# RoadlyInc/DSOPP

Hardware: AMD Instinct MI355X
Metric: Gauss-Newton iters/sec (7-KF window, 2k active pts) (higher is better)
Workload: dtype f64; 1 GPU; C1: 7-KF window, 2000 active points per GPU (2000 total, 2000 on rank 0), 640x480, full clique, production LM settings; frames=7, points_per_gpu=2000, total_points=2000, parallelism=single GPU, exchange=none, ranks=1

## Files before the change

### dsopp_amd/csrc/pba.hip

```cpp
#include <algorithm>
#include <chrono>
#include <cstdlib>
#include <map>
#include <memory>
#include <mutex>

#include "host_linalg.hpp"
#include "pba_solve_kernels.hpp"
#include "pba_solve_combined.hpp"
#include "pba_schur_two_stage.hpp"
#include "depth_map_kernels.hpp"
#include "point_status_kernels.hpp"
#include "depth_maps.hpp"
#include "activation_kernels.hpp"
#include "immature_set.hpp"
#include "semantic_observation_kernels.hpp"

namespace dsopp_hip {
namespace {

struct ResidualTable {
  DeviceBuffer<uint8_t> status, cand, fej_valid, snap_status;
  DeviceBuffer<double> energy;
  int n = 0, snap_n = 0;
// ... 924 lines not shown
  a.st = w.d_state.ptr;
  const bool combined = fused && fused->combined;
  const size_t reduce_count = combined ? w.combCount() : w.reduceCount();
  a.comb = combined ? w.d_reduce.ptr : nullptr;
  a.comb_lambda = fused ? fused->comb_lambda : 0.0;
  if (combined && mode == ReduceMode::kAccumulateOnly && w.comb_copies_active > 1) {
    a.comb_copies = w.comb_copies_active;
    a.comb_copy_first = static_cast<int>(w.combCopyFirst());
    a.comb_copy_stride = static_cast<int>(w.combCopyStride());
  }
  a.scalars = mode == ReduceMode::kDecideOnly ? w.d_reduce.ptr + reduce_count : w.d_scalars.ptr;
  a.n_sweep_blocks = w.n_sweep_blocks;
  a.total_blocks = a.n_schur_blocks + F * F;
  a.scalars_out = mode == ReduceMode::kAccumulateOnly ? w.d_reduce.ptr + reduce_count : nullptr;
  const bool grouped_tail = mode == ReduceMode::kAccumulateOnly && w.allreduce != nullptr;
  a.scalars_out_groups = grouped_tail ? kScalarGroups : 0;
  static_assert(4 * kScalarGroups <= kSchurThreads, "one workgroup writes the grouped tail");
  if (fused) a.prm = fused->prm;
  if (fused && fused->scalars) a.scalars = fused->scalars;
  a.ctrl_host = fused ? fused->ctrl_host : nullptr;
  a.dbg = w.dbg_stamps ? w.dbg_stamps.get() + 24 : nullptr;
  return a;
}

void launchReduceSchur(W &w, bool for_marg, const LmControl *ctrl, const FusedReduce *fused = nullptr, ReduceMode mode = ReduceMode::kFused) {
  const int K = w.K(), F = w.F();
  hipStream_t st = w.sr.stream;
  if (!fused && !for_marg && !ctrl && w.deterministic) {
    launchTwoStage(w, nullptr, 0, 0.0, true, nullptr);
    allreduceIfNeeded(w, w.d_reduce.ptr, w.reduceCount());
    return;
  }
  ensureDynamicLds(reinterpret_cast<const void *>(reduceSchurKernel), w.sr.device, 96 * 1024);
  const ReduceSchurArgs a = makeReduceSchurArgs(w, for_marg, ctrl, fused, mode);
  const size_t reduce_count = (fused && fused->combined) ? w.combCount() : w.reduceCount();
  const bool grouped_tail = mode == ReduceMode::kAccumulateOnly && w.allreduce != nullptr;
  const size_t decide_smem = kDecideSmemBytes;
  if (mode == ReduceMode::kDecideOnly) {
    timedLaunch(w, DSOPP_HIP_KERNEL_ACCEPT,
                [&] { decideApplyKernel<<<std::max(1, a.n_schur_blocks), kSchurThreads, decide_smem, st>>>(a); });
    HIP_CHECK(hipGetLastError());
    return;
  }
  timedLaunch(w, DSOPP_HIP_KERNEL_SCHUR, [&] {
    reduceSchurKernel<<<a.n_schur_blocks + F * F + (a.scalars_out ? 1 : 0), kSchurThreads, std::max(schurSmemBytes(K), decide_smem), st>>>(
        a.ctrl, a.schur_table, a.pc, a.partials, a.pair_first_block, a.pair_num_blocks, a.n_schur_blocks, a.F, a);
  });
  HIP_CHECK(hipGetLastError());
  allreduceIfNeeded(w, w.d_reduce.ptr, reduce_count + (mode == ReduceMode::kAccumulateOnly ? (grouped_tail ? 4 * kScalarGroups : 4) : 0));
  (void)K;
}

SolveArgs makeSolveArgs(W &w) {
  SolveArgs a;
  a.frames = w.d_frames.ptr;
  a.st = w.d_state.ptr;
  a.pc = w.d_pc.ptr;
  a.Hpp_raw = w.dHppRaw();
  a.bpp_raw = w.dbppRaw();
  a.Hpp_out = w.d_Hpp.ptr;
  a.Hsc_copy = w.d_Hpp.ptr + static_cast<size_t>(w.K()) * w.K();
  a.bpp_out = w.d_bpp.ptr;
  a.Hsc = w.dHsc();
  a.bsc = w.dbsc();
  a.use_marginal = w.marg_nonzero ? 1 : 0;
  a.Hm = w.d_Hm.ptr;
  a.bm = w.d_bm.ptr;
  a.step = w.d_step.ptr;
  a.lambda = 0;
  a.affine_reg[0] = w.opt.affine_brightness_regularizer[0];
  a.affine_reg[1] = w.opt.affine_brightness_regularizer[1];
  a.fixed_reg = w.opt.fixed_state_regularizer;
  a.energy_marginalized = w.energy_marginalized;
  a.F = w.F();
  a.fej = w.fej() ? 1 : 0;
  a.do_solve = 1;
  a.store_system = 0;
  a.add_priors = 1;
  return a;
}

size_t solveSmemBytes(int K) {
  const size_t N = static_cast<size_t>(K) + 1;
  return (N * (N + 1) + 4 * static_cast<size_t>(K) + 32 + 38 * static_cast<size_t>(kMaxFrames)) * sizeof(double);
}

void launchAssemble(W &w, double lambda, bool do_solve, bool add_priors, bool store_system) {
  ensureDynamicLds(reinterpret_cast<const void *>(assembleSolveKernel), w.sr.device, 150 * 1024);
  SolveArgs a = makeSolveArgs(w);
  a.lambda = lambda;
  a.do_solve = do_solve ? 1 : 0;
  a.add_priors = add_priors ? 1 : 0;
  a.store_system = store_system ? 1 : 0;
  timedLaunch(w, do_solve ? DSOPP_HIP_KERNEL_ASSEMBLE_SOLVE : DSOPP_HIP_KERNEL_ASSEMBLE,
              [&] { assembleSolveKernel<<<1, kSolveThreads, solveSmemBytes(w.K()), w.sr.stream>>>(a); });
  if (do_solve && !w.fej()) {
    pairSetupKernel<<<1, kMaxFrames * kMaxFrames, 0, w.sr.stream>>>(w.d_frames.ptr, w.d_state.ptr, w.d_pc.ptr, w.F(), 0, nullptr);
  }
  HIP_CHECK(hipGetLastError());
}

void launchTwoStage(W &w, const LmControl *ctrl, int ublk_parity, double lambda, bool dense = false, double *group_sums = nullptr) {
  const int F = w.F();
  hipStream_t st = w.sr.stream;
  using TwoStageKernel = void (*)(TwoStageArgs);
  static const TwoStageKernel kernels[6] = {nullptr, schurTwoStageKernel<2>, schurTwoStageKernel<2>, schurTwoStageKernel<3>, schurTwoStageKernel<4>,
                                            schurTwoStageKernel<5>};
  const int tpw = twoStageTilesPerWave(F);
  if (tpw < 1 || tpw > kMaxTilesPerWave) fail(DSOPP_HIP_ERR_CAPACITY, "window of %d frames exceeds the Schur kernel's tile budget", F);
  const TwoStageKernel two_stage_kernel = kernels[tpw];
  ensureDynamicLds(reinterpret_cast<const void *>(two_stage_kernel), w.sr.device, 96 * 1024);
  const int n_chunks = w.opt.optimize_idepths ? w.n_schur_blocks : 0;
  const int n_wgs = std::max(1, std::min(512, n_chunks));
  w.d_schur_partials.reserve(std::max<size_t>(1, static_cast<size_t>(n_wgs)) * static_cast<size_t>(twoStagePartialCount(F)), 0, st);
  w.d_pair_out.reserve(static_cast<size_t>(kMaxFrames) * kMaxFrames * kPairOut, 0, st);
  TwoStageArgs a;
  a.frames = w.d_frames.ptr;
  a.pc = w.d_pc.ptr;
  a.schur_table = w.d_schur_table.ptr;
  a.partials = w.d_partials.ptr;
  a.dbg = w.dbg_stamps ? w.dbg_stamps.get() + 32 : nullptr;
  a.pair_first_block = w.d_pair_first.ptr;
  a.pair_num_blocks = w.d_pair_count.ptr;
  a.ctrl = ctrl;
  a.schur_partials = w.d_schur_partials.ptr;
  a.pair_out = w.d_pair_out.ptr;
  a.F = F;
  a.n_chunks = n_chunks;
  a.n_schur_wgs = n_wgs;
  a.ublk_parity = ublk_parity;
  a.group_sums = group_sums;
  a.n_sweep_blocks = w.n_sweep_blocks;
  CombineArgs c;
  c.pc = w.d_pc.ptr;
  c.schur_partials = w.d_schur_partials.ptr;
  c.pair_out = w.d_pair_out.ptr;
  c.ctrl = ctrl;
  c.lambda = lambda;
  c.comb = w.d_reduce.ptr;
  c.dense = dense ? w.d_reduce.ptr : nullptr;
  c.F = F;
  c.n_schur_wgs = n_wgs;
  const size_t pair_smem = (48 + 64 + kPairBlk + 8 * 48) * sizeof(double);
  timedLaunch(w, DSOPP_HIP_KERNEL_SCHUR, [&] {
    two_stage_kernel<<<n_wgs + F * F + (group_sums ? kScalarGroups : 0), kSchurThreads, std::max(twoStageSmemBytes(F), pair_smem), st>>>(a);
    combineSystemKernel<<<static_cast<unsigned>((twoStagePartialCount(F) + kCombineEntries - 1) / kCombineEntries), kCombineEntries * kCombineSlices, 0, st>>>(c);
  });
  HIP_CHECK(hipGetLastError());
}

int solveResidentWorkgroups(W &w, bool wide) {
  static std::map<std::pair<int, size_t>, int> cache;
  static std::mutex mu;
  const size_t smem = solveSmemBytes(w.K());
  std::lock_guard<std::mutex> lock(mu);
  const auto key = std::make_pair(w.sr.device * 2 + (wide ? 1 : 0), smem);
  auto it = cache.find(key);
  if (it != cache.end()) return it->second;
  int per_cu = 0, cus = 0;
  if (wide)
    HIP_CHECK(hipOccupancyMaxActiveBlocksPerMultiprocessor(&per_cu, solveCombinedKernel<512>, 512, smem));
  else
    HIP_CHECK(hipOccupancyMaxActiveBlocksPerMultiprocessor(&per_cu, solveCombinedKernel<256>, 256, smem));
  HIP_CHECK(hipDeviceGetAttribute(&cus, hipDeviceAttributeMultiprocessorCount, w.sr.device));
  const int n = std::max(2, per_cu * cus);
  cache[key] = n;
  return n;
// ... 2688 lines not shown
```

### dsopp_amd/csrc/pba_solve_combined.hpp

```cpp
#pragma once
#include "pba_solve_kernels.hpp"

namespace dsopp_hip {

struct SolveCombArgs {
  const FrameDev *frames;
  WindowState *st;
  PairConst *pc;
  const double *comb;
  int comb_copies = 1;
  int comb_copy_first = 0, comb_copy_stride = 0;
  const double *Hm, *bm;
  const double *HmPacked = nullptr;
  double *step;
  LmControl *ctrl;
  double lambda;
  double affine_reg[2];
  double fixed_reg;
  double energy_marginalized;
  int F;
  int fej;
  int use_marginal;
  long long *dbg_stamps;
  const LmControl *dec_in = nullptr;
  const double *dec_scalars = nullptr;
  const SchurBlock *dec_table = nullptr;
  int dec_blocks = 0;
  int dec_groups = 0;
  LmParams dec_prm;
  unsigned *bs_ticket = nullptr;
  double *bs_hand = nullptr;
  double *bs_hand_next = nullptr;
  int bs_parity = 0;
  int dec_chunks = 0;
  unsigned bs_ticket_base = 0;
  int *bs_fault = nullptr;
  const unsigned *arrive = nullptr;
  unsigned arrive_target = 0;
  int fused_first = 0;
};
__device__ __forceinline__ bool waitForReducers(const unsigned *arrive, unsigned target, bool patient, int *fault) {
  const long long t0 = wall_clock64();
  for (;;) {
    const unsigned v = __hip_atomic_load(glb(arrive), __ATOMIC_RELAXED, __HIP_MEMORY_SCOPE_AGENT);
    if (static_cast<int>(v - target) >= 0) return true;
    if (patient)
      __builtin_amdgcn_s_sleep(24);
    else
      __builtin_amdgcn_s_sleep(1);
    if (wall_clock64() - t0 > 200000000ll) {
      if (fault) __hip_atomic_store(fault, 1, __ATOMIC_RELAXED, __HIP_MEMORY_SCOPE_SYSTEM);
      return false;
    }
  }
}
__host__ __device__ inline double kHandOverSentinel() {
  union {
    unsigned long long u;
    double d;
  } c;
  c.u = 0x7FF8D50FF00DBEEFull;
  return c.d;
}
constexpr int kMaxCombCopies = 4;
#define SC_STAMP(i) do { if (kStamps && a.dbg_stamps && tid == 0) a.dbg_stamps[i] = wall_clock64(); } while (0)

__device__ __forceinline__ void combBlockDecode(int b, int &bi, int &bj) {
  int r = static_cast<int>((__fsqrt_rn(8.0f * static_cast<float>(b) + 1.0f) - 1.0f) * 0.5f);
  if ((r + 1) * (r + 2) / 2 <= b) ++r;
  if (r * (r + 1) / 2 > b) --r;
  bi = r;
  bj = b - r * (r + 1) / 2;
}

template <int THREADS, int COPIES, bool FUSED>
__device__ __forceinline__ void solveCombinedBody(char *smem_raw, unsigned *bs_ticket_p, double *bs_hand_next_p, const LmControl *dec_in_p,
                                                  const double *dec_scalars_p, const double *comb_p, const FrameDev *frames_p, WindowState *st_p,
                                                  int F_p, const SolveCombArgs &a, const double *t_fused) {
  const int F = F_p, K = kBlk * F;
  const int N = K + 1;
  const int ld = N + 1;
  double *A = reinterpret_cast<double *>(smem_raw);
  double *pv = A + N * ld;
  double *xs = pv + K;
  double *Linv = xs + K + 16;
  double *epsl = Linv + 36 * kMaxFrames;
  double *stpl = epsl + K;
  double *ab0l = stpl + K;
  const int tid = threadIdx.x;
  const int wave = tid >> 6, lane = tid & 63;
  const long long sc_t_entry = (kStamps && a.dbg_stamps) ? wall_clock64() : 0;

  int c_active = 1, c_relin = 0;
  double lam = a.lambda;
  const bool decides = dec_in_p != nullptr;
  double dec_eps = 0, dec_step = 0;
  int dec_accept = 0;
  const bool ticketed = FUSED || bs_ticket_p != nullptr;
  const unsigned vblock_f = FUSED ? blockIdx.x - static_cast<unsigned>(a.fused_first) : 0u;
  unsigned ticket_raw = 0;
  if (!FUSED && ticketed && tid == 0) {
    auto tp = glb(bs_ticket_p);
    asm volatile("" : "+v"(tp));
    ticket_raw = __hip_atomic_fetch_add(tp, 1u, __ATOMIC_RELAXED, __HIP_MEMORY_SCOPE_AGENT);
  }
  if (ticketed && tid < kBlk * kMaxFrames) bs_hand_next_p[tid] = kHandOverSentinel();
  const void DSOPP_CONSTANT *any_words = (const void DSOPP_CONSTANT *)__builtin_amdgcn_kernarg_segment_ptr();
  const LmControl DSOPP_CONSTANT *cin_src = dec_in_p ? (const LmControl DSOPP_CONSTANT *)dec_in_p : (const LmControl DSOPP_CONSTANT *)any_words;
  static_assert(sizeof(SolveCombArgs) >= sizeof(LmControl) && sizeof(SolveCombArgs) >= 4 * sizeof(double), "the argument block stands in for an absent control block / scalar block");
  static_assert(sizeof(LmControl) == 6 * sizeof(double) + 8 * sizeof(int), "LmControl changed: extend the scalar copy below");
  LmControl cin;
  cin.lambda = cin_src->lambda;
  cin.energy = cin_src->energy;
  cin.cand_prior = cin_src->cand_prior;
  cin.idepth_sq = cin_src->idepth_sq;
  cin.frame_state_sq = cin_src->frame_state_sq;
  cin.frame_step_sq = cin_src->frame_step_sq;
  cin.n_valid = cin_src->n_valid;
  cin.converged = cin_src->converged;
  cin.active = cin_src->active;
  cin.linear_system_valid = cin_src->linear_system_valid;
  cin.iteration = cin_src->iteration;
  cin.need_final_setup = cin_src->need_final_setup;
  cin.pending = cin_src->pending;
  cin.relin = cin_src->relin;
  const double DSOPP_CONSTANT *t_src =
      (!FUSED && dec_scalars_p) ? (const double DSOPP_CONSTANT *)dec_scalars_p : (const double DSOPP_CONSTANT *)any_words;
  double t_early[4] = {t_src[0], t_src[1], t_src[2], t_src[3]};
  asm volatile("" : "+s"(cin.lambda), "+s"(cin.energy), "+s"(cin.cand_prior), "+s"(cin.idepth_sq), "+s"(cin.frame_state_sq), "+s"(cin.frame_step_sq),
               "+s"(cin.n_valid), "+s"(cin.converged), "+s"(cin.active), "+s"(cin.linear_system_valid), "+s"(cin.iteration),
               "+s"(cin.need_final_setup), "+s"(cin.pending), "+s"(cin.relin), "+s"(t_early[0]), "+s"(t_early[1]), "+s"(t_early[2]), "+s"(t_early[3])
               : "s"(a.pc), "s"(a.Hm), "s"(a.bm), "s"(a.HmPacked), "s"(a.step), "s"(a.ctrl), "s"(a.fej), "s"(a.use_marginal), "s"(a.dec_table),
               "s"(a.dec_blocks), "s"(a.dec_groups), "s"(a.bs_hand), "s"(a.bs_parity), "s"(a.dec_chunks), "s"(a.bs_ticket_base), "s"(a.comb_copies),
               "s"(a.comb_copy_first), "s"(a.comb_copy_stride), "s"(a.lambda), "s"(a.affine_reg[0]), "s"(a.affine_reg[1]), "s"(a.fixed_reg),
               "s"(a.energy_marginalized));
  __shared__ unsigned s_vblock;
  bool main_wg = FUSED ? vblock_f == 0 : (ticketed || blockIdx.x == 0);
  const bool reducers_build = FUSED && cin.active && !cin.linear_system_valid;
  struct {
    int valid;
    Rigid T0;
    double fxr, fyr, cxr, cyr, fxt, fyt, cxt, cyt, exposure_r, exposure_t;
  } pp;
  pp.valid = 0;
  const bool fast_refresh = a.fej != 0;
  auto requestPairInputs = [&] {
    if (fast_refresh && tid < F * F) {
      const int r = tid / F, t = tid - F * (tid / F);
      const PairConst &P = a.pc[r * kMaxFrames + t];
      pp.valid = P.valid;
#pragma unroll
      for (int i = 0; i < 3; ++i) {
#pragma unroll
        for (int j = 0; j < 3; ++j) pp.T0.R[3 * i + j] = P.T0rel[4 * i + j];
        pp.T0.t[i] = P.T0rel[4 * i + 3];
      }
      const FrameDev &fr = frames_p[r];
      const FrameDev &ft = frames_p[t];
      pp.fxr = fr.fx;
      pp.fyr = fr.fy;
      pp.cxr = fr.cx;
      pp.cyr = fr.cy;
      pp.fxt = ft.fx;
      pp.fyt = ft.fy;
      pp.cxt = ft.cx;
      pp.cyt = ft.cy;
      pp.exposure_r = fr.exposure;
      pp.exposure_t = ft.exposure;
    }
  };
  double eps_c = 0, ab0_c = 0, rhs_c = 0, bm_c = 0;
  int fixed_c = 0, tomarg_c = 0;
// ... 227 lines not shown
              break;
            }
          }
        }
        stp[tid] = v;
      }
      __syncthreads();
      if (s_timed_out) return;
      const double damp = 1.0 / (1.0 + s_dec_out.lambda);
      auto finish = [&](const double (&rw)[NS][kBlk], double bd, double ih, hbm_f64 *dst) {
        double d = 0;
    #pragma unroll
        for (int q = 0; q < NS; ++q) {
          const double *sq = stp + kBlk * (sub + 4 * q);
    #pragma unroll
          for (int c = 0; c < kBlk; ++c) d += rw[q][c] * sq[c];
        }
        d += dppMove<0xB1>(d);
        d += dppMove<0x4E>(d);
        if (sub == 0 && dst) *dst = -((bd - d) * damp * ih);
      };
    #pragma unroll
      for (int u = 0; u < kPre; ++u) finish(rows[u], bdv[u], ihv[u], dstp[u]);
      for (int p = static_cast<int>(vblock) - 1 + kPre * W; p < n_pass; p += W) {
        double rw[NS][kBlk], bd = 0, ih = 0;
        hbm_f64 *dst = nullptr;
    #pragma unroll
        for (int q = 0; q < NS; ++q)
    #pragma unroll
          for (int c = 0; c < kBlk; ++c) rw[q][c] = 0;
        fetch(p, rw, bd, ih, dst);
        finish(rw, bd, ih, dst);
      }
      };
      if (THREADS < 512)
        backSubstitute(std::integral_constant<int, 2>{});
      else if (F <= 12)
        backSubstitute(std::integral_constant<int, 3>{});
      else
        backSubstitute(std::integral_constant<int, 4>{});
      return;
    }
    if (cin.pending && tid < K) {
      if (dec_accept) {
        dec_eps += dec_step;
        st_p->eps[tid >> 3][tid & 7] = dec_eps;
      }
      st_p->step[tid >> 3][tid & 7] = 0;
    }
    if (tid == 64) *a.ctrl = s_dec_out;
    if (!s_dec_proceed) return;
    c_active = 1;
    c_relin = s_dec_out.relin;
    lam = s_dec_out.lambda;
  } else if (a.ctrl) {
    c_active = a.ctrl->active;
    c_relin = a.ctrl->relin;
    lam = a.ctrl->lambda;
  }
  if (decides) eps_c = dec_eps;
  SC_STAMP(0);
  if (kStamps && a.dbg_stamps && tid == 0) a.dbg_stamps[7] = sc_t_entry;
  asm volatile("" : "+v"(fixed_c), "+v"(tomarg_c), "+v"(c_active), "+v"(c_relin));
  int prior_kind = 0;
  double pd_c = 0;
  if (tid < K) {
    if (!tomarg_c) prior_kind = fixed_c ? 1 : ((tid & 7) >= 6 ? 2 : 0);
    pd_c = prior_kind == 1 ? a.fixed_reg : (prior_kind == 2 ? ((tid & 7) == 6 ? a.affine_reg[0] : a.affine_reg[1]) : 0.0);
    xs[tid] = eps_c;
    epsl[tid] = eps_c;
    Linv[tid] = pd_c;
    if ((tid & 7) >= 6) ab0l[2 * (tid >> 3) + (tid & 7) - 6] = ab0_c;
  }
  ldsBarrier();
  SC_STAMP(10);
  if (!c_active || c_relin) return;
  if (FUSED) {
    __shared__ int s_system_there;
    if (tid == 0) s_system_there = (!reducers_build || waitForReducers(a.arrive, a.arrive_target, false, a.bs_fault)) ? 1 : 0;
    ldsBarrier();
    if (!s_system_there) return;
    SC_STAMP(16);
    if (tid < K) rhs_c = __hip_atomic_load(glb(comb_p) + combBlockCount(F) * 64 + tid, __ATOMIC_RELAXED, __HIP_MEMORY_SCOPE_AGENT);
    loadBatch(0);
  }
  const double *prior_diag = Linv;
  const int in_row = (tid >> 3) & 7, in_col = tid & 7;
  double *const A_thr = A + in_row * ld + in_col;
  auto storeBatch = [&](int base) {
    int blk = __builtin_amdgcn_readfirstlane((base + tid) >> 6);
    int bi, bj;
    combBlockDecode(blk, bi, bj);
    bi = __builtin_amdgcn_readfirstlane(bi);
    bj = __builtin_amdgcn_readfirstlane(bj);
    const int n_blocks = n_entries >> 6;
#pragma unroll
    for (int u = 0; u < kBatch; ++u) {
      if (blk < n_blocks) {
        const int blk_off = __builtin_amdgcn_readfirstlane(8 * bi * ld + 8 * bj);
        const double v = hv[u] + hm[u];
        if (bi != bj) {
          A_thr[blk_off] = v;
        } else if (in_col <= in_row) {
          double vd = v;
          if (in_row == in_col) {
            const int row = 8 * bi + in_row;
            vd += prior_diag[row] * (1.0 + lam);
            pv[row] = vd + 10.0;
          }
          A_thr[blk_off] = vd;
        }
      }
      blk += THREADS / 64;
      bj += THREADS / 64;
      while (bj > bi) {
        bj -= bi + 1;
        ++bi;
      }
    }
  };
  storeBatch(0);
  for (int base = kBatch * THREADS; base < n_entries; base += kBatch * THREADS) {
    loadBatch(base);
    storeBatch(base);
  }
  SC_STAMP(11);
  if (tid < K) {
    double v = rhs_c;
    if (prior_kind == 1)
      v += a.fixed_reg * eps_c;
    else if (prior_kind == 2)
      v += ((tid & 7) == 6 ? a.affine_reg[0] : a.affine_reg[1]) * (ab0_c + eps_c);
    if (a.use_marginal) {
      double s = 0;
      for (int k = 0; k < K; ++k) s += a.Hm[tid * K + k] * xs[k];
      v += bm_c + s;
    }
    A[K * ld + tid] = v;
  }
  if (tid == 0) A[K * ld + K] = 0;
  ldsBarrier();
  SC_STAMP(1);
  if (main_wg) requestPairInputs();

  choleskyAugmented<THREADS>(A, pv, Linv, F, tid, a.dbg_stamps);
  SC_STAMP(2);
  if (ticketed) requestTailInputs();
  if (wave == 0) {
    backSubstituteWave(A, Linv, xs, F, lane);
    SC_STAMP(6);
  }
  __syncthreads();
  if (tid < K) {
    const double x = xs[tid];
    stpl[tid] = -x;
    if (a.bs_hand) __hip_atomic_store(a.bs_hand + tid, x, __ATOMIC_RELAXED, __HIP_MEMORY_SCOPE_AGENT);
    a.step[tid] = x;
    st_p->step[tid >> 3][tid & 7] = -x;
  }
  SC_STAMP(3);
  double part = 0, nstate = 0, nstep = 0;
  auto priorMath = [&] {
    if (!a.ctrl || !prior_thread) return;
    const double xc = epsl[pc] + stpl[pc];
    if (a.use_marginal) {
      double sacc = 0;
      for (int k = 0; k < K; ++k) sacc += a.Hm[pc * K + k] * (epsl[k] + stpl[k]);
      part += bm_p * xc + 0.5 * xc * sacc;
    }
    if ((pc & 7) >= 6) {
      const double ab = ab0_p + xc;
      part += 0.5 * ab * ((pc & 7) == 6 ? a.affine_reg[0] : a.affine_reg[1]) * ab;
    }
    nstate = epsl[pc] * epsl[pc] + ((pc & 7) >= 6 ? ab0_p * ab0_p : 0.0);
    nstep = stpl[pc] * stpl[pc];
  };
  if (fast_refresh) {
    ldsBarrier();
    Rigid *E = reinterpret_cast<Rigid *>(A);
    if (tid < 2 * F) {
      const int f = tid < F ? tid : tid - F;
      const double sign = tid < F ? 1.0 : -1.0;
      double xi[6];
#pragma unroll
      for (int i = 0; i < 6; ++i) xi[i] = sign * (epsl[kBlk * f + i] + stpl[kBlk * f + i]);
      E[tid] = rigidExp(xi);
    }
    ldsBarrier();
    asm volatile("" : "+v"(pp.valid));
    if (tid < F * F && pp.valid) {
      const int r = tid / F, t = tid - F * (tid / F);
      PairConst &P = a.pc[r * kMaxFrames + t];
      const Rigid T_tr = rigidMul(E[F + t], rigidMul(pp.T0, E[r]));
      const double ifx = 1.0 / pp.fxr, ify = 1.0 / pp.fyr;
      const double k02 = -pp.cxr * ifx, k12 = -pp.cyr * ify;
      double U[12];
#pragma unroll
      for (int i = 0; i < 3; ++i) {
        U[4 * i + 0] = T_tr.R[3 * i + 0] * ifx;
        U[4 * i + 1] = T_tr.R[3 * i + 1] * ify;
        U[4 * i + 2] = T_tr.R[3 * i + 0] * k02 + T_tr.R[3 * i + 1] * k12 + T_tr.R[3 * i + 2];
        U[4 * i + 3] = T_tr.t[i];
      }
#pragma unroll
      for (int j = 0; j < 4; ++j) {
        P.M[0 + j] = pp.fxt * U[0 + j] + pp.cxt * U[8 + j];
        P.M[4 + j] = pp.fyt * U[4 + j] + pp.cyt * U[8 + j];
        P.M[8 + j] = U[8 + j];
      }
      const double a_r = ab0l[2 * r] + epsl[kBlk * r + 6] + stpl[kBlk * r + 6];
      const double a_t = ab0l[2 * t] + epsl[kBlk * t + 6] + stpl[kBlk * t + 6];
      P.s = (pp.exposure_t / pp.exposure_r) * exp(a_t - a_r);
      P.b_t = ab0l[2 * t + 1] + epsl[kBlk * t + 7] + stpl[kBlk * t + 7];
      P.b_r = ab0l[2 * r + 1] + epsl[kBlk * r + 7] + stpl[kBlk * r + 7];
    }
    priorMath();
  } else {
    ldsBarrier();
    priorMath();
  }
  SC_STAMP(4);
  if (a.ctrl && K <= 64) {
    if (wave == 1) {
      part = waveSum(part);
      nstate = waveSum(nstate);
      nstep = waveSum(nstep);
      if (tid == 64) {
        a.ctrl->cand_prior = a.energy_marginalized + part;
        a.ctrl->frame_state_sq = nstate;
        a.ctrl->frame_step_sq = nstep;
        a.ctrl->pending = 1;
      }
    }
  } else if (a.ctrl) {
    part = waveSum(part);
    nstate = waveSum(nstate);
    nstep = waveSum(nstep);
    ldsBarrier();
    if ((tid & 63) == 0) {
      xs[tid >> 6] = part;
      xs[THREADS / 64 + (tid >> 6)] = nstate;
      xs[2 * (THREADS / 64) + (tid >> 6)] = nstep;
    }
    ldsBarrier();
    if (tid == 64) {
      constexpr int kWaves = THREADS / 64;
      double total = a.energy_marginalized, s_state = 0, s_step = 0;
      for (int w = 0; w < kWaves; ++w) {
        total += xs[w];
        s_state += xs[kWaves + w];
        s_step += xs[2 * kWaves + w];
      }
      a.ctrl->cand_prior = total;
      a.ctrl->frame_state_sq = s_state;
      a.ctrl->frame_step_sq = s_step;
      a.ctrl->pending = 1;
    }
  }
  SC_STAMP(5);
}

template <int THREADS, int COPIES = 1>
__global__ void __launch_bounds__(THREADS, 1) solveCombinedKernel(unsigned *bs_ticket_p, double *bs_hand_next_p, const LmControl *dec_in_p,
                                                                  const double *dec_scalars_p, const double *comb_p, const FrameDev *frames_p,
                                                                  WindowState *st_p, int F_p, SolveCombArgs a) {
  extern __shared__ __attribute__((aligned(16))) char smem_raw[];
  solveCombinedBody<THREADS, COPIES, false>(smem_raw, bs_ticket_p, bs_hand_next_p, dec_in_p, dec_scalars_p, comb_p, frames_p, st_p, F_p, a, nullptr);
}

template <int THREADS>
__global__ void __launch_bounds__(kSchurThreads) reduceSolveFusedKernel(const LmControl *ctrl_p, const SchurBlock *table_p, const PairConst *pc_p,
                                                                        const double *partials_p, const int *pair_first_p, const int *pair_num_p,
                                                                        int n_schur_blocks_p, int F_p, ReduceSchurArgs ra, SolveCombArgs sa) {
  static_assert(THREADS == 256 || THREADS == kSchurThreads, "the solve body's two instantiations");
  extern __shared__ __attribute__((aligned(16))) char smem_raw[];
  const int n_reducers = n_schur_blocks_p + F_p * F_p + 1;
  if (static_cast<int>(blockIdx.x) < n_reducers) {
    reduceSchurBody<true>(smem_raw, ctrl_p, table_p, pc_p, partials_p, pair_first_p, pair_num_p, n_schur_blocks_p, F_p, ra);
    __builtin_amdgcn_s_waitcnt(0);
    __syncthreads();
    if (threadIdx.x == 0) __hip_atomic_fetch_add(glb(const_cast<unsigned *>(sa.arrive)), 1u, __ATOMIC_RELAXED, __HIP_MEMORY_SCOPE_AGENT);
    return;
  }
  __shared__ double s_sums[4];
  if (static_cast<int>(blockIdx.x) == n_reducers) {
    double *lds = reinterpret_cast<double *>(smem_raw);
    double v[4] = {0, 0, 0, 0};
    for (int b = threadIdx.x; b < ra.n_sweep_blocks; b += kSchurThreads) {
      const double *p = partials_p + static_cast<size_t>(b) * kPartial + 44;
      v[0] += p[0];
      v[1] += p[1];
      v[2] += p[2];
      v[3] += p[3];
    }
#pragma unroll
    for (int e = 0; e < 4; ++e) lds[e * (kSchurThreads + 2) + threadIdx.x] = v[e];
    __syncthreads();
    if (threadIdx.x < 4) {
      double sacc = 0;
      for (int j = 0; j < kSchurThreads; ++j) sacc += lds[threadIdx.x * (kSchurThreads + 2) + j];
      s_sums[threadIdx.x] = sacc;
    }
    __syncthreads();
  }
  if (static_cast<int>(threadIdx.x) >= THREADS) return;
  solveCombinedBody<THREADS, 1, true>(smem_raw, nullptr, sa.bs_hand_next, ctrl_p, nullptr, sa.comb, sa.frames, sa.st, F_p, sa, s_sums);
}

}
```

### dsopp_amd/csrc/pba_solve_kernels.hpp

```cpp
#pragma once
#include <cstddef>
#include <type_traits>
#include "pba_kernels.hpp"

namespace dsopp_hip {


struct LmParams {
  double function_tolerance, parameter_tolerance;
  double decrease_on_accept, increase_on_reject;
  double lambda0;
  int max_iterations, min_iterations;
  int force_accept;
  int use_reduced_scalars;
};

constexpr int kSchurLandmarks = 64;
constexpr int kSchurThreads = 512;
constexpr int kPairBlk = 144;

__host__ __device__ inline int schurRowStride(int Kp) {
  return ((Kp + 15) / 32) * 32 + 16;
}

// ... 645 lines not shown

__global__ void __launch_bounds__(kSchurThreads) reduceSchurKernel(const LmControl *ctrl_p, const SchurBlock *table_p, const PairConst *pc_p,
                                                                   const double *partials_p, const int *pair_first_p, const int *pair_num_p,
                                                                   int n_schur_blocks_p, int F_p, ReduceSchurArgs a) {
  extern __shared__ __attribute__((aligned(16))) char smem_raw[];
  reduceSchurBody<false>(smem_raw, ctrl_p, table_p, pc_p, partials_p, pair_first_p, pair_num_p, n_schur_blocks_p, F_p, a);
}

__global__ void __launch_bounds__(kSchurThreads) decideApplyKernel(ReduceSchurArgs a) {
  extern __shared__ __attribute__((aligned(16))) char smem_raw[];
  long long dbg_unused[2] = {0, 0};
  ApplyRegs ar;
  ar.pending = 0;
  ar.publish = 0;
  fusedDecideApply(a, reinterpret_cast<double *>(smem_raw), dbg_unused, ar);
  applyDecision(a, ar);
}

__global__ void clearSchurKernel(double *buf, int n, const LmControl *ctrl) {
  if (ctrl && (!ctrl->active || ctrl->linear_system_valid)) return;
  const int i = blockIdx.x * blockDim.x + threadIdx.x;
  if (i < n) buf[i] = 0;
}

constexpr int kSolveThreads = 256;

struct SolveArgs {
  const FrameDev *frames;
  WindowState *st;
  PairConst *pc;
  const double *Hpp_raw, *bpp_raw;
  double *Hsc;
  const double *bsc;
  double *Hpp_out, *bpp_out;
  double *Hsc_copy = nullptr;
  const double *Hm, *bm;
  double *step;
  double lambda;
  double affine_reg[2];
  double fixed_reg;
  double energy_marginalized;
  int F;
  int fej;
  int do_solve;
  int store_system;
  int add_priors;
  int use_marginal;
};

__device__ inline double priorEnergyBlock(const SolveArgs &a, bool with_step, double *lds , int tid) {
  const int F = a.F, K = kBlk * F;
  for (int c = tid; c < K; c += kSolveThreads) lds[c] = a.st->eps[c >> 3][c & 7] + (with_step ? a.st->step[c >> 3][c & 7] : 0.0);
  __syncthreads();
  double part = 0;
  for (int c = tid; c < K; c += kSolveThreads) {
    if (a.use_marginal) {
      double s = 0;
      for (int k = 0; k < K; ++k) s += a.Hm[c * K + k] * lds[k];
      part += a.bm[c] * lds[c] + 0.5 * lds[c] * s;
    }
    if ((c & 7) >= 6) {
      const double ab = a.st->ab0[c >> 3][(c & 7) - 6] + lds[c];
      part += 0.5 * ab * a.affine_reg[(c & 7) - 6] * ab;
    }
  }
  part = waveSum(part);
  __syncthreads();
  if ((tid & 63) == 0) lds[K + (tid >> 6)] = part;
  __syncthreads();
  double total = a.energy_marginalized;
  for (int w = 0; w < kSolveThreads / 64; ++w) total += lds[K + w];
  __syncthreads();
  return total;
}

__host__ __device__ constexpr int lowIdx(int i, int j) { return i * (i + 1) / 2 + j; }

__device__ __forceinline__ double readLane(double v, int src_lane) {
  const int lo = __builtin_amdgcn_readlane(__double2loint(v), src_lane);
  const int hi = __builtin_amdgcn_readlane(__double2hiint(v), src_lane);
  return __hiloint2double(hi, lo);
}

template <int THREADS>
__device__ __forceinline__ void choleskyAugmented(double *A, const double *pv, double *Linv, int F, int tid, long long *stamps) {
  const int K = kBlk * F;
  const int N = K + 1;
  const int ld = N + 1;
  const int wave = tid >> 6, lane = tid & 63;
  auto factorAndPanel = [&](int kb) {
    const int k0 = kb * kBlk;
    const int row = k0 + lane;
    const bool valid = row < N;
    double c[kBlk], invd[kBlk], lj[28];
    {
      const double *src = A + (valid ? row : k0) * ld + k0;
#pragma unroll
      for (int j = 0; j < kBlk; ++j) c[j] = src[j];
    }
    double guard[kBlk];
#pragma unroll
    for (int k = 0; k < kBlk; ++k) guard[k] = 1e-30 * pv[min(k0 + k, K - 1)];
    int e = 0;
    auto rsqrtRefined = [](double d) {
      const double hd = 0.5 * d;
      double inv = __builtin_amdgcn_rsq(d);
      inv = fma(inv, fma(-hd * inv, inv, 0.5), inv);
      inv = fma(inv, fma(-hd * inv, inv, 0.5), inv);
      return inv;
    };
#pragma unroll
    for (int k = 0; k < kBlk; ++k) {
      const double d = readLane(c[k], k);
      const bool okp = d > guard[k];
      double inv = rsqrtRefined(d);
      inv = okp ? inv : 0.0;
      invd[k] = inv;
      const double l = c[k] * inv;
      c[k] = l;
#pragma unroll
      for (int j = k + 1; j < kBlk; ++j) {
        const double ljk = readLane(l, j);
        lj[e++] = ljk;
        c[j] -= l * ljk;
      }
    }
    if (valid) {
      double *dst = A + row * ld + k0;
#pragma unroll
      for (int j = 0; j < kBlk; ++j)
        if (lane >= kBlk || j <= lane) dst[j] = c[j];
    }
    for (int r2 = row + 64; r2 < N; r2 += 64) {
      double v[kBlk];
#pragma unroll
      for (int j = 0; j < kBlk; ++j) v[j] = A[r2 * ld + k0 + j];
      int e2 = 0;
#pragma unroll
      for (int k = 0; k < kBlk; ++k) {
        v[k] *= invd[k];
#pragma unroll
        for (int j = k + 1; j < kBlk; ++j) v[j] -= v[k] * lj[e2++];
      }
#pragma unroll
      for (int j = 0; j < kBlk; ++j) A[r2 * ld + k0 + j] = v[j];
    }
    if (lane == 0) {
#pragma unroll
      for (int cidx = 0; cidx < kBlk; ++cidx) Linv[kb * 36 + lowIdx(cidx, cidx)] = invd[cidx];
    }
  };
  long long cs_acc[4] = {0, 0, 0, 0}, cs_t = (kStamps && stamps) ? wall_clock64() : 0;
  auto csMark = [&](int slot) {
    if (kStamps && stamps) {
      const long long now = wall_clock64();
      cs_acc[slot] += now - cs_t;
      cs_t = now;
    }
  };
  if (wave == 0) factorAndPanel(0);
  ldsBarrier();
  csMark(2);
  for (int kb = 0; kb < F; ++kb) {
    const int k0 = kb * kBlk, k1 = k0 + kBlk, k2 = k1 + kBlk;
    if (kb + 1 < F) {
      const int n_el = (N - k1) * kBlk;
      for (int e = tid; e < n_el; e += THREADS) {
        const int row = k1 + (e >> 3), col = k1 + (e & 7);
        if (col > row) continue;
        const double *li = A + row * ld + k0, *lj = A + col * ld + k0;
        double sacc = 0;
#pragma unroll
        for (int c = 0; c < kBlk; ++c) sacc += li[c] * lj[c];
        A[row * ld + col] -= sacc;
      }
    }
    csMark(0);
    ldsBarrier();
    csMark(1);
    if (wave == 0) {
      if (kb + 1 < F) factorAndPanel(kb + 1);
      csMark(2);
    } else {
      const int t = tid - 64, tr = t >> 4, tc = t & 15;
      for (int row = k2 + tr; row < N; row += (THREADS - 64) / 16) {
        const double *li = A + row * ld + k0;
        double lic[kBlk];
#pragma unroll
        for (int c = 0; c < kBlk; ++c) lic[c] = li[c];
        for (int col = k2 + tc; col <= row; col += 16) {
          const double *lj = A + col * ld + k0;
          double sacc = 0;
#pragma unroll
          for (int c = 0; c < kBlk; ++c) sacc += lic[c] * lj[c];
          A[row * ld + col] -= sacc;
        }
      }
    }
    ldsBarrier();
    csMark(3);
  }
  if (kStamps && stamps && tid == 0) {
    for (int q = 0; q < 4; ++q) stamps[12 + q] = cs_acc[q];
  }
}

__device__ __forceinline__ void backSubstituteWave(const double *A, const double *Linv, double *xs, int F, int lane) {
  const int K = kBlk * F, ld = K + 2;
  auto run = [&](auto two_tag) {
    constexpr bool TWO = decltype(two_tag)::value;
    const int j0 = lane, j1 = lane + 64;
    double y0 = j0 < K ? A[K * ld + j0] : 0.0, y1 = (TWO && j1 < K) ? A[K * ld + j1] : 0.0;
    const double gi0 = j0 < K ? Linv[(j0 >> 3) * 36 + lowIdx(j0 & 7, j0 & 7)] : 0.0;
    const double gi1 = (TWO && j1 < K) ? Linv[(j1 >> 3) * 36 + lowIdx(j1 & 7, j1 & 7)] : 0.0;
    double g0[kBlk], g1[kBlk], n0[kBlk], n1[kBlk];
    auto loadBlock = [&](int kb, double *o0, double *o1) {
#pragma unroll
      for (int c = 0; c < kBlk; ++c) {
        o0[c] = A[(kb * kBlk + c) * ld + j0];
        if (TWO) o1[c] = j1 < K ? A[(kb * kBlk + c) * ld + j1] : 0.0;
      }
    };
    auto sweepBlocks = [&](auto upper_tag, int kb_from, int kb_to) {
      constexpr bool UPPER = decltype(upper_tag)::value;
      for (int kb = kb_from; kb >= kb_to; --kb) {
        if (kb > 0) {
#pragma unroll
          for (int c = 0; c < kBlk; ++c) {
            n0[c] = A[((kb - 1) * kBlk + c) * ld + j0];
            if (UPPER) n1[c] = j1 < K ? A[((kb - 1) * kBlk + c) * ld + j1] : 0.0;
          }
        }
        double xo[kBlk];
#pragma unroll
        for (int c = kBlk - 1; c >= 0; --c) {
          const int k = kb * kBlk + c;
          const double xk = UPPER ? readLane(y1 * gi1, k & 63) : readLane(y0 * gi0, k);
          xo[c] = xk;
          y0 -= g0[c] * xk;
          if (UPPER) y1 -= g1[c] * xk;
        }
        if (lane == 0) {
#pragma unroll
          for (int c = 0; c < kBlk; ++c) xs[kb * kBlk + c] = xo[c];
        }
#pragma unroll
        for (int c = 0; c < kBlk; ++c) {
          g0[c] = n0[c];
          if (UPPER) g1[c] = n1[c];
        }
      }
    };
    loadBlock(F - 1, g0, g1);
    if (TWO) {
      sweepBlocks(std::true_type{}, F - 1, 8);
      sweepBlocks(std::false_type{}, 7, 0);
    } else {
      sweepBlocks(std::false_type{}, F - 1, 0);
    }
  };
  if (K > 64)
    run(std::true_type{});
  else
    run(std::false_type{});
}

__global__ void __launch_bounds__(kSolveThreads, 1) assembleSolveKernel(SolveArgs a) {
  extern __shared__ __attribute__((aligned(16))) char smem_raw[];
  const int F = a.F, K = kBlk * F;
  const int N = K + 1;
  const int ld = N + 1;
  double *A = reinterpret_cast<double *>(smem_raw);
  double *pv = A + N * ld;
  double *xs = pv + K;
  double *Linv = xs + K + 16;
  const int tid = threadIdx.x;
  const double lam = a.lambda;
  double eps_c = 0, ab0_c = 0, bpp_c = 0, bsc_c = 0, bm_c = 0;
  int fixed_c = 0, tomarg_c = 0;
  if (tid < K) {
    const int f = tid >> 3, i = tid & 7;
    eps_c = a.st->eps[f][i];
    fixed_c = a.frames[f].fixed;
    tomarg_c = a.frames[f].to_marginalize;
    ab0_c = a.st->ab0[f][i < 6 ? 0 : i - 6];
    bpp_c = a.bpp_raw[tid];
    bsc_c = a.bsc[tid];
// ... 9 lines not shown
#pragma unroll
    for (int u = 0; u < kTileBatch; ++u) {
      int tile = base + u, tr0 = 0;
      while (tile >= tr0 + 1) {
        tile -= tr0 + 1;
        ++tr0;
      }
      const int row = 16 * tr0 + tile_r, col = 16 * tile + tile_c;
      const bool in = (base + u) < n_tiles && row < K && col < K;
      rows[u] = in ? row : -1;
      cols[u] = col;
      const int rc = min(row, K - 1), cc = min(col, K - 1);
      hp[u] = a.Hpp_raw[rc * K + cc];
      hs[u] = a.Hsc[min(rc, cc) * K + max(rc, cc)];
      hm[u] = 0;
    }
    if (a.use_marginal) {
#pragma unroll
      for (int u = 0; u < kTileBatch; ++u) {
        const int rc = min(rows[u] < 0 ? 0 : rows[u], K - 1), cc = min(cols[u], K - 1);
        hm[u] = a.Hm[rc * K + cc];
      }
    }
  };
  loadBatch(0);
  asm volatile("" : "+v"(fixed_c), "+v"(tomarg_c));
  int prior_kind = 0;
  if (tid < K) {
    if (a.add_priors && !tomarg_c) prior_kind = fixed_c ? 1 : ((tid & 7) >= 6 ? 2 : 0);
    const double pd_c = prior_kind == 1 ? a.fixed_reg : (prior_kind == 2 ? a.affine_reg[(tid & 7) - 6] : 0.0);
    xs[tid] = eps_c;
    prior_diag[tid] = pd_c;
  }
  __syncthreads();
  const double sc = -1.0 / (1.0 + lam);
  auto storeBatch = [&]() {
#pragma unroll
    for (int u = 0; u < kTileBatch; ++u) {
      const int row = rows[u], col = cols[u];
      if (row < 0) continue;
      double v = hp[u];
      if (row == col) v += prior_diag[row];
      if (a.store_system) {
        a.Hpp_out[row * K + col] = v;
        a.Hpp_out[col * K + row] = a.Hpp_raw[col * K + row] + (row == col ? prior_diag[row] : 0.0);
        if (col < row) a.Hsc[row * K + col] = hs[u];
        if (a.Hsc_copy && col <= row) {
          a.Hsc_copy[row * K + col] = hs[u];
          a.Hsc_copy[col * K + row] = hs[u];
        }
      }
      if (col <= row) {
        if (row == col) v += v * lam;
        A[row * ld + col] = v + sc * hs[u] + hm[u];
      }
    }
  };
  storeBatch();
  for (int base = kTileBatch; base < n_tiles; base += kTileBatch) {
    loadBatch(base);
    storeBatch();
  }
  __syncthreads();
  if (tid < K) {
    const int c = tid;
    double v = bpp_c;
    if (prior_kind == 1)
      v += a.fixed_reg * eps_c;
    else if (prior_kind == 2)
      v += a.affine_reg[(c & 7) - 6] * (ab0_c + eps_c);
    if (a.store_system) a.bpp_out[c] = v;
    v += sc * bsc_c;
    if (a.use_marginal) {
      double s = 0;
      for (int k = 0; k < K; ++k) s += a.Hm[c * K + k] * xs[k];
      v += bm_c + s;
    }
    A[K * ld + c] = v;
    pv[c] = A[c * ld + c] + 10.0;
  }
  if (tid == 0) A[K * ld + K] = 0;
  if (!a.do_solve) return;
  __syncthreads();
  choleskyAugmented<kSolveThreads>(A, pv, Linv, F, tid, nullptr);
  if (tid < 64) backSubstituteWave(A, Linv, xs, F, tid);
  __syncthreads();
  if (tid < K) {
    const double x = xs[tid];
    a.step[tid] = x;
    a.st->step[tid >> 3][tid & 7] = -x;
  }
  __syncthreads();
  Rigid *E = reinterpret_cast<Rigid *>(A);
  if (tid < 2 * F) E[tid] = frameIncrement(a.st, tid % F, tid < F ? 1.0 : -1.0);
  __syncthreads();
  if (tid < F * F && a.fej) refreshPairCurrent(a.frames, a.st, a.pc, tid / F, tid % F, E[tid / F], E[F + tid % F]);
}

__global__ void backsubKernel(const FrameDev *__restrict__ frames, const SchurBlock *__restrict__ table, const double *__restrict__ step,
                              double lambda, int F, const LmControl *ctrl, int ublk_parity, int gate_on_pending) {
  if (ctrl) {
    if (!ctrl->active || (gate_on_pending && !ctrl->pending)) return;
    lambda = ctrl->lambda;
  }
  const SchurBlock be = table[blockIdx.x];
  const FrameDev &fr = frames[be.r];
  const int i = be.offset + threadIdx.x;
  if (threadIdx.x >= kSchurLandmarks || i >= fr.n) return;
  const uint8_t flg = fr.flags[i];
  if (flg & kFlagMarginalized) return;
  if (flg & kFlagIllConditioned) return;
  double d = 0;
  for (int t = 0; t < F; ++t) {
    if (t != be.r && fr.status[t] == nullptr) continue;
    const double *src = fr.ublk + (static_cast<size_t>(ublk_parity) * kMaxFrames + t) * ublkPlane(fr.cap) + static_cast<size_t>(i) * kUblk;
#pragma unroll
    for (int c = 0; c < kBlk; ++c) d += src[c] * step[kBlk * t + c];
  }
  const double s = (fr.b_d[i] - d) * (1.0 / (1.0 + lambda)) * fr.inv_hdd[i];
  fr.idepth_step[i] = -s;
}

__global__ void energyReduceKernel(const double *__restrict__ partials, int n_blocks, double *out) {
  __shared__ double lds[(256 / 64) * 2];
  double v[2] = {0, 0};
  for (int b = threadIdx.x; b < n_blocks; b += blockDim.x) {
    v[0] += partials[static_cast<size_t>(b) * kPartial + 44];
    v[1] += partials[static_cast<size_t>(b) * kPartial + 45];
  }
  blockSum<2, 256>(v, lds);
  if (threadIdx.x == 0) {
    out[0] = v[0];
    out[1] = v[1];
  }
}

__global__ void acceptLandmarksKernel(const FrameDev *__restrict__ frames, const SchurBlock *__restrict__ table, int F, int accept,
                                      double *norms) {
  __shared__ double lds[(kSchurThreads / 64) * 2];
  const SchurBlock be = table[blockIdx.x];
  const FrameDev &fr = frames[be.r];
  const int i = be.offset + threadIdx.x;
  double v[2] = {0, 0};
  if (threadIdx.x < kSchurLandmarks && i < fr.n) {
    if (accept) {
      const double id = fr.idepth[i], st = fr.idepth_step[i];
      v[0] = id * id;
      v[1] = st * st;
      fr.idepth[i] = id + st;
    }
    fr.idepth_step[i] = 0;
    for (int t = 0; t < F; ++t) {
      if (fr.status[t] == nullptr || i >= fr.n_res[t]) continue;
      if (accept)
        fr.status[t][i] = fr.cand[t][i];
      else
        fr.cand[t][i] = fr.status[t][i];
    }
  }
  blockSum<2, kSchurThreads>(v, lds);
  if (threadIdx.x == 0 && accept) {
    atomicAdd(&norms[0], v[0]);
    atomicAdd(&norms[1], v[1]);
  }
}

__global__ void acceptFramesKernel(WindowState *st, int F, int accept, double *norms ) {
  __shared__ double lds[4];
  const int c = threadIdx.x;
  double v[2] = {0, 0};
  if (c < kBlk * F) {
    const int f = c >> 3, a = c & 7;
    if (accept) {
// ... 161 lines not shown
```

Measured before the change: 26500 GN iterations/s.

## Compute solution columns on helper waves during blocked Cholesky, skipping back-substitution

Helper waves, including extra waves added to the fused solve workgroup, now build columns of the inverse factor block by block alongside the blocked Cholesky factorization. They accumulate the solution directly and emit each step component. This removes the serial single-wave back-substitution after factorization. In exchange it adds register pressure, extra LDS scratch, and wave-level exchanges, plus a larger launch footprint in the fused kernel.

```diff
diff --git a/dsopp_amd/csrc/pba.hip b/dsopp_amd/csrc/pba.hip
--- a/dsopp_amd/csrc/pba.hip
+++ b/dsopp_amd/csrc/pba.hip
@@ -1030,7 +1030,7 @@
 
 size_t solveSmemBytes(int K) {
   const size_t N = static_cast<size_t>(K) + 1;
-  return (N * (N + 1) + 4 * static_cast<size_t>(K) + 32 + 38 * static_cast<size_t>(kMaxFrames)) * sizeof(double);
+  return (N * (N + 1) + 4 * static_cast<size_t>(K) + 32 + 38 * static_cast<size_t>(kMaxFrames) + (kSchurThreads - 64)) * sizeof(double);
 }
 
 void launchAssemble(W &w, double lambda, bool do_solve, bool add_priors, bool store_system) {
diff --git a/dsopp_amd/csrc/pba_solve_combined.hpp b/dsopp_amd/csrc/pba_solve_combined.hpp
--- a/dsopp_amd/csrc/pba_solve_combined.hpp
+++ b/dsopp_amd/csrc/pba_solve_combined.hpp
@@ -73,7 +73,7 @@
   bj = b - r * (r + 1) / 2;
 }
 
-template <int THREADS, int COPIES, bool FUSED>
+template <int THREADS, int COPIES, bool FUSED, int WG = THREADS>
 __device__ __forceinline__ void solveCombinedBody(char *smem_raw, unsigned *bs_ticket_p, double *bs_hand_next_p, const LmControl *dec_in_p,
                                                   const double *dec_scalars_p, const double *comb_p, const FrameDev *frames_p, WindowState *st_p,
                                                   int F_p, const SolveCombArgs &a, const double *t_fused) {
@@ -87,7 +87,9 @@
   double *epsl = Linv + 36 * kMaxFrames;
   double *stpl = epsl + K;
   double *ab0l = stpl + K;
+  double *colx = ab0l + 2 * kMaxFrames;
   const int tid = threadIdx.x;
+  const bool extra = WG > THREADS && tid >= THREADS;
   const int wave = tid >> 6, lane = tid & 63;
   const long long sc_t_entry = (kStamps && a.dbg_stamps) ? wall_clock64() : 0;
 
@@ -481,7 +483,7 @@
     if (!s_system_there) return;
     SC_STAMP(16);
     if (tid < K) rhs_c = __hip_atomic_load(glb(comb_p) + combBlockCount(F) * 64 + tid, __ATOMIC_RELAXED, __HIP_MEMORY_SCOPE_AGENT);
-    loadBatch(0);
+    if (!extra) loadBatch(0);
   }
   const double *prior_diag = Linv;
   const int in_row = (tid >> 3) & 7, in_col = tid & 7;
@@ -518,10 +520,12 @@
       }
     }
   };
-  storeBatch(0);
-  for (int base = kBatch * THREADS; base < n_entries; base += kBatch * THREADS) {
-    loadBatch(base);
-    storeBatch(base);
+  if (!extra) {
+    storeBatch(0);
+    for (int base = kBatch * THREADS; base < n_entries; base += kBatch * THREADS) {
+      loadBatch(base);
+      storeBatch(base);
+    }
   }
   SC_STAMP(11);
   if (tid < K) {
@@ -540,24 +544,37 @@
   if (tid == 0) A[K * ld + K] = 0;
   ldsBarrier();
   SC_STAMP(1);
-  if (main_wg) requestPairInputs();
-
-  choleskyAugmented<THREADS>(A, pv, Linv, F, tid, a.dbg_stamps);
-  SC_STAMP(2);
-  if (ticketed) requestTailInputs();
-  if (wave == 0) {
-    backSubstituteWave(A, Linv, xs, F, lane);
+  constexpr bool kColumns = WG > THREADS;
+  if (!kColumns && main_wg) requestPairInputs();
+
+  auto stepOut = [&](int q, double x) {
+    stpl[q] = -x;
+    if (a.bs_hand) __hip_atomic_store(a.bs_hand + q, x, __ATOMIC_RELAXED, __HIP_MEMORY_SCOPE_AGENT);
+    a.step[q] = x;
+    st_p->step[q >> 3][q & 7] = -x;
+  };
+  if (kColumns) {
+    choleskyAugmentedImpl<THREADS, WG, true>(A, pv, Linv, F, tid, a.dbg_stamps, colx, true, stepOut);
+    if (main_wg) requestPairInputs();
+    SC_STAMP(2);
+    if (ticketed) requestTailInputs();
+    ldsBarrier();
     SC_STAMP(6);
-  }
-  __syncthreads();
-  if (tid < K) {
-    const double x = xs[tid];
-    stpl[tid] = -x;
-    if (a.bs_hand) __hip_atomic_store(a.bs_hand + tid, x, __ATOMIC_RELAXED, __HIP_MEMORY_SCOPE_AGENT);
-    a.step[tid] = x;
-    st_p->step[tid >> 3][tid & 7] = -x;
-  }
-  SC_STAMP(3);
+    if (extra) return;
+  } else {
+    choleskyAugmented<THREADS>(A, pv, Linv, F, tid, a.dbg_stamps);
+    SC_STAMP(2);
+    if (ticketed) requestTailInputs();
+    if (wave == 0) {
+      backSubstituteWave(A, Linv, xs, F, lane);
+      SC_STAMP(6);
+    }
+    __syncthreads();
+    if (tid < K) stepOut(tid, xs[tid]);
+    SC_STAMP(3);
+    ldsBarrier();
+  }
+  if (kColumns) SC_STAMP(3);
   double part = 0, nstate = 0, nstep = 0;
   auto priorMath = [&] {
     if (!a.ctrl || !prior_thread) return;
@@ -575,7 +592,6 @@
     nstep = stpl[pc] * stpl[pc];
   };
   if (fast_refresh) {
-    ldsBarrier();
     Rigid *E = reinterpret_cast<Rigid *>(A);
     if (tid < 2 * F) {
       const int f = tid < F ? tid : tid - F;
@@ -615,7 +631,6 @@
     }
     priorMath();
   } else {
-    ldsBarrier();
     priorMath();
   }
   SC_STAMP(4);
@@ -702,8 +717,8 @@
     }
     __syncthreads();
   }
-  if (static_cast<int>(threadIdx.x) >= THREADS) return;
-  solveCombinedBody<THREADS, 1, true>(smem_raw, nullptr, sa.bs_hand_next, ctrl_p, nullptr, sa.comb, sa.frames, sa.st, F_p, sa, s_sums);
+  if (THREADS < kSchurThreads && static_cast<int>(threadIdx.x) >= THREADS && static_cast<int>(blockIdx.x) != n_reducers) return;
+  solveCombinedBody<THREADS, 1, true, kSchurThreads>(smem_raw, nullptr, sa.bs_hand_next, ctrl_p, nullptr, sa.comb, sa.frames, sa.st, F_p, sa, s_sums);
 }
 
 }
diff --git a/dsopp_amd/csrc/pba_solve_kernels.hpp b/dsopp_amd/csrc/pba_solve_kernels.hpp
--- a/dsopp_amd/csrc/pba_solve_kernels.hpp
+++ b/dsopp_amd/csrc/pba_solve_kernels.hpp
@@ -751,8 +751,10 @@
   return __hiloint2double(hi, lo);
 }
 
-template <int THREADS>
-__device__ __forceinline__ void choleskyAugmented(double *A, const double *pv, double *Linv, int F, int tid, long long *stamps) {
+template <int THREADS, int WG, bool COLUMNS, class Emit>
+__device__ __forceinline__ void choleskyAugmentedImpl(double *A, const double *pv, double *Linv, int F, int tid, long long *stamps, double *ex, bool cols,
+                                                      Emit emit) {
+  static_assert(WG >= THREADS && (WG == 256 || WG == 512), "three or seven helper waves behind the panel wave (first_block)");
   const int K = kBlk * F;
   const int N = K + 1;
   const int ld = N + 1;
@@ -827,12 +829,106 @@
       cs_t = now;
     }
   };
+  constexpr int H = WG / 64 - 1;
+  constexpr int NS = (8 + H - 1) / H;
+  const bool helper_cols = COLUMNS && cols;
+  const bool helper = helper_cols && wave > 0;
+  const int cg = lane >> 3, rho = lane & 7;
+  double cs[NS][kBlk - 1], cx[NS];
+#pragma unroll
+  for (int sl = 0; sl < NS; ++sl) {
+    cx[sl] = 0;
+#pragma unroll
+    for (int i = 0; i < kBlk - 1; ++i) cs[sl][i] = 0;
+  }
+  const int first_block = H == 7 ? (wave >= 5 ? 7 - wave : (wave == 4 ? 6 : 6 - wave)) : wave - 1;
+  double *exw = ex + (wave > 0 ? wave - 1 : 0) * 64;
+  auto exchange = [&](int sl, int kb, double (&t)[kBlk]) {
+    double own = 0;
+#pragma unroll
+    for (int i = 1; i < kBlk; ++i) own = i == kb ? cs[sl][i - 1] : own;
+    exw[lane] = -own;
+    __builtin_amdgcn_s_waitcnt(0xC07F);
+    __builtin_amdgcn_wave_barrier();
+#pragma unroll
+    for (int c = 0; c < kBlk; ++c) t[c] = exw[kBlk * cg + c];
+    __builtin_amdgcn_wave_barrier();
+  };
+  double t_last[kBlk];
+#pragma unroll
+  for (int c = 0; c < kBlk; ++c) t_last[c] = 0;
+  auto columnStep = [&](int kb, auto last_tag) {
+    constexpr bool LAST = decltype(last_tag)::value;
+    const int k0 = kb * kBlk;
+    if (first_block > kb) return;
+    const double *lrow = A + rho * ld + k0;
+#pragma unroll
+    for (int sl = 0; sl < NS; ++sl) {
+      const int b = first_block + H * sl;
+      if (b > kb || b >= F) continue;
+      double ld_[28], iv[kBlk];
+      {
+        int e = 0;
+#pragma unroll
+        for (int c = 0; c < kBlk; ++c) {
+          iv[c] = Linv[kb * 36 + lowIdx(c, c)];
+#pragma unroll
+          for (int c2 = 0; c2 < c; ++c2) ld_[e++] = A[(k0 + c) * ld + k0 + c2];
+        }
+      }
+      double t[kBlk];
+      if (b == kb) {
+#pragma unroll
+        for (int c = 0; c < kBlk; ++c) t[c] = c == cg ? 1.0 : 0.0;
+      } else if (LAST && sl == 0) {
+#pragma unroll
+        for (int c = 0; c < kBlk; ++c) t[c] = t_last[c];
+      } else {
+        exchange(sl, kb, t);
+      }
+      double z[kBlk];
+      {
+        int e = 0;
+#pragma unroll
+        for (int c = 0; c < kBlk; ++c) {
+          double acc = t[c];
+#pragma unroll
+          for (int c2 = 0; c2 < c; ++c2) acc = fma(-ld_[e++], z[c2], acc);
+          z[c] = acc * iv[c];
+        }
+      }
+      double x = cx[sl];
+#pragma unroll
+      for (int c = 0; c < kBlk; ++c) x = fma(z[c], A[K * ld + k0 + c], x);
+      cx[sl] = x;
+      if (!LAST) __builtin_amdgcn_sched_barrier(0);
+      auto updateRange = [&](auto lo_tag, auto hi_tag) {
+        constexpr int LO = decltype(lo_tag)::value, HI = decltype(hi_tag)::value;
+#pragma unroll
+        for (int i = LO; i < HI; ++i) {
+          const double *lr = lrow + kBlk * min(i, F - 1) * ld;
+          double sacc = cs[sl][i - 1];
+#pragma unroll
+          for (int c = 0; c < kBlk; ++c) sacc = fma(lr[c], z[c], sacc);
+          cs[sl][i - 1] = sacc;
+        }
+        __builtin_amdgcn_sched_barrier(0);
+      };
+      if (!LAST) {
+        if (kb < 3) updateRange(std::integral_constant<int, 1>{}, std::integral_constant<int, 4>{});
+        updateRange(std::integral_constant<int, 4>{}, std::integral_constant<int, 6>{});
+        updateRange(std::integral_constant<int, 6>{}, std::integral_constant<int, kBlk>{});
+        if (sl == 0 && kb + 2 == F) exchange(0, kb + 1, t_last);
+      }
+    }
+  };
   if (wave == 0) factorAndPanel(0);
   ldsBarrier();
   csMark(2);
-  for (int kb = 0; kb < F; ++kb) {
+  auto blockStep = [&](int kb, auto has_next_tag) {
+    constexpr bool HAS_NEXT = decltype(has_next_tag)::value;
     const int k0 = kb * kBlk, k1 = k0 + kBlk, k2 = k1 + kBlk;
-    if (kb + 1 < F) {
+    if ((WG == THREADS || tid < THREADS) && (HAS_NEXT || kb + 1 < F)) {
       const int n_el = (N - k1) * kBlk;
       for (int e = tid; e < n_el; e += THREADS) {
         const int row = k1 + (e >> 3), col = k1 + (e & 7);
@@ -848,30 +944,51 @@
     ldsBarrier();
     csMark(1);
     if (wave == 0) {
-      if (kb + 1 < F) factorAndPanel(kb + 1);
+      if (HAS_NEXT || kb + 1 < F) factorAndPanel(kb + 1);
       csMark(2);
     } else {
-      const int t = tid - 64, tr = t >> 4, tc = t & 15;
-      for (int row = k2 + tr; row < N; row += (THREADS - 64) / 16) {
-        const double *li = A + row * ld + k0;
-        double lic[kBlk];
-#pragma unroll
-        for (int c = 0; c < kBlk; ++c) lic[c] = li[c];
-        for (int col = k2 + tc; col <= row; col += 16) {
-          const double *lj = A + col * ld + k0;
-          double sacc = 0;
-#pragma unroll
-          for (int c = 0; c < kBlk; ++c) sacc += lic[c] * lj[c];
-          A[row * ld + col] -= sacc;
-        }
-      }
+      if (WG == THREADS || tid < THREADS) {
+        const int t = tid - 64, tr = t >> 4, tc = t & 15;
+        for (int row = k2 + tr; row < N; row += (THREADS - 64) / 16) {
+          const double *li = A + row * ld + k0;
+          double lic[kBlk];
+#pragma unroll
+          for (int c = 0; c < kBlk; ++c) lic[c] = li[c];
+          for (int col = k2 + tc; col <= row; col += 16) {
+            const double *lj = A + col * ld + k0;
+            double sacc = 0;
+#pragma unroll
+            for (int c = 0; c < kBlk; ++c) sacc += lic[c] * lj[c];
+            A[row * ld + col] -= sacc;
+          }
+        }
+      }
+      if (helper) columnStep(kb, std::false_type{});
     }
     ldsBarrier();
     csMark(3);
+  };
+  if (helper_cols) {
+    for (int kb = 0; kb + 1 < F; ++kb) blockStep(kb, std::true_type{});
+  } else {
+    for (int kb = 0; kb < F; ++kb) blockStep(kb, std::false_type{});
   }
   if (kStamps && stamps && tid == 0) {
     for (int q = 0; q < 4; ++q) stamps[12 + q] = cs_acc[q];
   }
+  if (helper) {
+    columnStep(F - 1, std::true_type{});
+#pragma unroll
+    for (int sl = 0; sl < NS; ++sl) {
+      const int b = first_block + H * sl;
+      if (b < F && rho == 0) emit(kBlk * b + cg, cx[sl]);
+    }
+  }
+}
+
+template <int THREADS>
+__device__ __forceinline__ void choleskyAugmented(double *A, const double *pv, double *Linv, int F, int tid, long long *stamps) {
+  choleskyAugmentedImpl<THREADS, THREADS, false>(A, pv, Linv, F, tid, stamps, nullptr, false, [](int, double) {});
 }
 
 __device__ __forceinline__ void backSubstituteWave(const double *A, const double *Linv, double *xs, int F, int lane) {
@@ -1047,13 +1164,20 @@
   if (tid == 0) A[K * ld + K] = 0;
   if (!a.do_solve) return;
   __syncthreads();
-  choleskyAugmented<kSolveThreads>(A, pv, Linv, F, tid, nullptr);
-  if (tid < 64) backSubstituteWave(A, Linv, xs, F, tid);
-  __syncthreads();
-  if (tid < K) {
-    const double x = xs[tid];
-    a.step[tid] = x;
-    a.st->step[tid >> 3][tid & 7] = -x;
+  const bool by_columns = K <= 64;
+  double *ex = Linv + 36 * kMaxFrames;
+  choleskyAugmentedImpl<kSolveThreads, kSolveThreads, true>(A, pv, Linv, F, tid, nullptr, ex, by_columns, [&](int q, double x) {
+    a.step[q] = x;
+    a.st->step[q >> 3][q & 7] = -x;
+  });
+  if (!by_columns) {
+    if (tid < 64) backSubstituteWave(A, Linv, xs, F, tid);
+    __syncthreads();
+    if (tid < K) {
+      const double x = xs[tid];
+      a.step[tid] = x;
+      a.st->step[tid >> 3][tid & 7] = -x;
+    }
   }
   __syncthreads();
   Rigid *E = reinterpret_cast<Rigid *>(A);
```

New measurement: 28710 GN iterations/s (median of 6 runs). +8.3%, better.
